# SkyTNT/midi-model

Hardware: AMD Instinct MI355X
Metric: MIDI events/sec, training step (fwd+bwd+clip+AdamW), tv2o-medium, seq=2048 (higher is better)
Workload: dtype bf16; 1 GPU; tv2o-medium bf16 training step, per-GPU batch 16 x 2048 events x 8 tokens (BASELINE.json configs[1]); random-init weights, synthetic events; global_batch=16, seq_len=2048, parallelism=dp1, accumulate_grad_batches=1, optimizer=AdamW bf16-true + global-norm clip 1.0

## Files before the change

### include/midihip.h

```cpp
#ifndef MIDIHIP_H
#define MIDIHIP_H
#include <stdint.h>
#ifdef __cplusplus
extern "C" {
#endif

#define MH_F32 0
#define MH_BF16 1

#define MH_OK 0
#define MH_ERR_ARG (-1)
#define MH_ERR_LAUNCH (-2)
#define MH_ERR_UNSUPPORTED (-3)

const char* mh_last_error(void);
int mh_version(void);
int mh_ab_builds(void);
int mh_set_option(const char* name, int value);
int mh_get_option(const char* name);

int mh_gemm_nt(const void* A, int64_t lda, const void* B, int64_t ldb, void* C, int64_t ldc, const void* R,
               int64_t ldr, int64_t M, int64_t N, int64_t K, float alpha, float beta, int dtype, int splitk,
               void* workspace, void* stream);
int mh_gemm(const void* A, int64_t lda, int transA, const void* B, int64_t ldb, int transB, void* C, int64_t ldc,
// ... 28 lines not shown
int mh_scale_cols_batched(const int64_t* jobs, int njobs, int K, int dtype, void* stream);
int mh_gemm_splitk_reduce(const void* workspace, void* C, int64_t ldc, const void* R, int64_t ldr, int64_t M,
                          int64_t N, int splitk, float alpha, float beta, int dtype, void* stream);
#define MH_SKINNY_PLAIN 0
#define MH_SKINNY_GATEUP 1
int mh_gemm_skinny(const void* A, int64_t lda, const void* W, int64_t ldw, void* C, int64_t ldc, const void* R,
                   int64_t ldr, int mode, float norm_eps, const int64_t* row_ids, const int64_t* res_ids, int64_t M,
                   int64_t N, int64_t K, int dtype, void* stream);
int mh_transpose(const void* in, int64_t ldi, void* out, int64_t ldo, int64_t rows, int64_t cols, int dtype,
                 void* stream);

int mh_embed_sum_fwd(const int64_t* tok, const void* table, void* out, int64_t M, int T, int64_t V, int D,
                     int dtype, void* stream);
int mh_concat_tok_fwd(const void* hidden, const int64_t* tok, int64_t ldtok, const void* table, void* out,
                      int64_t M, int T, int64_t V, int D, int dtype, void* stream);
int mh_embed_scatter_bwd(const int64_t* tok, int64_t ldtok, int T, const void* dout, int rows_per_m, int jstride,
                         int j0, float* dtable_f32, int64_t M, int64_t V, int D, int64_t pad_id, int dtype,
                         void* stream);
int mh_embed_segment_bwd(const int64_t* src_rows, const int64_t* seg_start, const void* dout, int64_t ld,
                         float* dtable_f32, int64_t V, int D, int64_t n_occ, int64_t pad_id, int dtype, void* stream);
int mh_embed_segment_sum(const int64_t* src_rows, const int64_t* seg_start, const void* rows, int64_t ld, float* sum_f32,
                         int64_t ldsum, int64_t V, int D, int64_t n_occ, int dtype, void* stream);
int mh_embed_split_hi_lo(const float* s, void* hi, void* lo, int64_t n, int dtype, void* stream);
int mh_embed_table_norm_bwd(const void* t_hi, const void* t_lo, const void* e, const float* rstd, float* acc32, int64_t V, int D,
                            int64_t pad_id, int dtype, void* stream);
int mh_token_segments_chunk(void);
int mh_token_segments(const int64_t* tok, int64_t ldtok, int64_t n_rows, int n_cols, int64_t V, int64_t row_mul,
                      int64_t col_mul, int64_t add, int64_t* src_rows, int64_t* seg_start, int32_t* work, void* stream);
int mh_cast_from_f32(const float* src, void* dst, int64_t n, int accumulate, int dtype, void* stream);
int mh_copy_rows(const void* src, int64_t src_ld, void* dst, int64_t dst_ld, int64_t M, int D, int accumulate,
                 int dtype, void* stream);

int mh_collate_windows(const int16_t* tokens, int64_t n_events, const int64_t* win_start, const int64_t* win_len,
                       int64_t* out, int64_t B, int64_t L, int T, int64_t pad_id, void* stream);

int mh_augment_piece_stats(const int16_t* tokens, const int64_t* piece_off, int64_t n_pieces, const int32_t* tab,
                           int32_t* stats, void* stream);
int mh_augment_collate_windows(const int16_t* tokens, int64_t n_events, const int64_t* win_start, const int64_t* win_len,
                               const int64_t* win_piece, const int32_t* shifts, const int32_t* stats, const int32_t* tab,
                               int64_t* out, int64_t B, int64_t L, int T, int64_t pad_id, void* stream);

int mh_rmsnorm_fwd(const void* x, const void* w, void* y, float* rstd, int64_t M, int D, float eps, int dtype,
                   void* stream);
int mh_rmsnorm_bwd_blocks(int64_t M);
int mh_rmsnorm_bwd(const void* x, const void* w, const float* rstd, const void* dy, const void* dres, void* dx,
                   float* dw_partial, int64_t M, int D, int dtype, void* stream);
int mh_colsum(float* partial , int64_t nblk, void* out, int D, int accumulate, int dtype, void* stream);

int mh_rope(void* qkv, const float* cos_t, const float* sin_t, int64_t M, int64_t S, int64_t pos0, int H, int hd,
            int dir, int dtype, void* stream);

// ... 7 lines not shown
                const float* cos_t, const float* sin_t, int dtype, void* stream);
int mh_attn_bwd_o(const void* qkv, const void* o, const void* dout, const float* lse, float* delta, void* dqkv, int64_t B,
                  int64_t S, int H, float scale, const float* cos_t, const float* sin_t, int dtype, void* stream);
int mh_attn_bwd_o_scaled(const void* qkv, const void* o, const void* dout, const float* lse, float* delta, void* dqkv,
                         const float* rowscale, int64_t B, int64_t S, int H, float scale, const float* cos_t, const float* sin_t,
                         int dtype, void* stream);
int mh_attn_fwd_timeline(const void* qkv, void* o, float* lse, int64_t B, int64_t S, int H, float scale, int lazy,
                         uint32_t* stamps, void* stream);
int mh_attn_fwd_plain(const void* qkv, void* o, float* lse, int64_t B, int64_t S, int H, float scale, int dtype,
                      void* stream);
int mh_attn_bwd_plain(const void* qkv, const void* dout, const float* lse, const float* delta, void* dqkv, int64_t B,
                      int64_t S, int H, float scale, int dtype, void* stream);

int mh_tokattn_fwd(const void* qkv, void* o, int64_t N, int T, int H, float scale, const float* cos_t, const float* sin_t,
                   int dtype, void* stream);
int mh_tokattn_bwd(const void* qkv, const void* dout, void* dqkv, int64_t N, int T, int H, float scale, const float* cos_t,
                   const float* sin_t, int dtype, void* stream);
int mh_tokattn_bwd_scaled(const void* qkv, const void* dout, void* dqkv, const float* rowscale, int64_t N, int T, int H, float scale,
                          const float* cos_t, const float* sin_t, int dtype, void* stream);
int mh_tokattn_fwd_rows(const void* zc, const int64_t* ids, int64_t ldid, int64_t tab0, int64_t V, void* o, int64_t N, int H,
                        float scale, const float* cos_t, const float* sin_t, int dtype, void* stream);
int mh_tokattn_bwd_rows(const void* zc, const int64_t* ids, int64_t ldid, int64_t tab0, int64_t V, const void* dout, void* dz,
                        void* dz_hid, const float* rowscale, int64_t N, int H, float scale, const float* cos_t, const float* sin_t,
                        int dtype, void* stream);

int mh_swiglu_fwd(const void* gu, void* a, int64_t M, int I, int dtype, void* stream);
int mh_swiglu_bwd(const void* gu, const void* da, void* dgu, int64_t M, int I, int dtype, void* stream);

int mh_cross_entropy(const void* logits, int64_t ldl, const int64_t* target, float* row_loss, void* dlogits,
                     const float* scale_dev, int64_t* argmax_out, int64_t R, int V, int64_t ignore, int dtype,
                     void* stream);
int mh_sum_f32(const float* x, int64_t n, float* out, void* stream);
int mh_count_valid(const int64_t* target, int64_t n, int64_t ignore, float* count, float* inv, void* stream);

int mh_sumsq(const void* g, int64_t n, float* partial1024, float* out, int accumulate, int dtype, void* stream);
int mh_clip_coef(const float* sumsq, float max_norm, float* coef, float* norm, void* stream);
int mh_adamw(void* p, const void* g, void* m, void* v, int64_t n, float lr, float beta1, float beta2, float eps,
             float weight_decay, float bias_corr1, float bias_corr2, const float* coef_dev, int dtype, void* stream);
int mh_adamw_master(float* p32, void* p_lo, const float* g32, float* m, float* v, int64_t n, float lr, float beta1,
                    float beta2, float eps, float weight_decay, float bias_corr1, float bias_corr2, const float* coef_dev,
                    int dtype_lo, void* stream);
int mh_grad_fold_f32(const void* src, float* dst, int64_t n, int accumulate, int dtype, void* stream);

int mh_kv_append(void* qkv, const float* cos_t, const float* sin_t, void* kcache, void* vcache, int64_t B, int H,
                 int hd, int64_t Lmax, int64_t pos, const int32_t* pos_dev, int dtype, void* stream);
int mh_attn_decode(const void* qkv, const void* kcache, const void* vcache, void* o, int64_t B, int H, int hd,
                   int64_t Lmax, int64_t len, float scale, const int32_t* pos_dev, int dtype, void* stream);
// ... 43 lines not shown
```

### midi-model_amd/csrc/attention_small.hip

```cpp
#include "common.h"

#define DISPATCH_T(dtype, CALL)                                    \
  do {                                                             \
    if ((dtype) == MH_BF16) { using T = bf16; CALL; }              \
    else if ((dtype) == MH_F32) { using T = float; CALL; }         \
    else { mh_set_error("bad dtype %d", (int)(dtype)); return MH_ERR_ARG; } \
  } while (0)

template <typename T> __device__ inline void ld4(const T* p, float (&o)[4]);
template <> __device__ inline void ld4<float>(const float* p, float (&o)[4]) {
  f32x4 v = *reinterpret_cast<const f32x4*>(p);
  o[0] = v[0]; o[1] = v[1]; o[2] = v[2]; o[3] = v[3];
}
template <> __device__ inline void ld4<bf16>(const bf16* p, float (&o)[4]) {
  bf16x4 v = *reinterpret_cast<const bf16x4*>(p);
  o[0] = (float)v[0]; o[1] = (float)v[1]; o[2] = (float)v[2]; o[3] = (float)v[3];
}
template <typename T> __device__ inline void st4(T* p, const float (&o)[4]);
template <> __device__ inline void st4<float>(float* p, const float (&o)[4]) {
  *reinterpret_cast<f32x4*>(p) = f32x4{o[0], o[1], o[2], o[3]};
}
template <> __device__ inline void st4<bf16>(bf16* p, const float (&o)[4]) {
  bf16x4 v;
  v[0] = (bf16)o[0]; v[1] = (bf16)o[1]; v[2] = (bf16)o[2]; v[3] = (bf16)o[3];
// ... 40 lines not shown
template <typename T>
__device__ inline void rope4(float (&x)[4], const float (&c)[2], const float (&s)[2], float dir, bool round) {
#pragma unroll
  for (int e = 0; e < 2; ++e) {
    const float x1 = x[e], x2 = x[e + 2], sn = dir * s[e];
    const float r1 = x1 * c[e] - x2 * sn, r2 = x2 * c[e] + x1 * sn;
    x[e] = round ? rnd<T>(r1) : r1;
    x[e + 2] = round ? rnd<T>(r2) : r2;
  }
}

template <typename T>
__device__ inline void rope_row(float (&x)[4], const float* rope_c, const float* rope_s, int t, int lane, float dir,
                                bool round) {
  const float rc[2] = {rope_c[t * 128 + 2 * lane], rope_c[t * 128 + 2 * lane + 1]};
  const float rs[2] = {rope_s[t * 128 + 2 * lane], rope_s[t * 128 + 2 * lane + 1]};
  rope4<T>(x, rc, rs, dir, round);
}

struct TokRows {
  const int64_t* ids;
  int64_t ldid, tab0;
  int V;
};
template <int TN>
__device__ inline int tok_row_lane(const TokRows& tr, int64_t n, int lane) {
  int id = 0;
  if (lane >= 1 && lane < TN) id = (int)tr.ids[n * tr.ldid + lane - 1];
  return id < 0 ? 0 : (id >= tr.V ? tr.V - 1 : id);
}

template <typename T, int TN, bool IND = false>
__global__ __launch_bounds__(256) void tokattn_fwd_kernel(const T* __restrict__ qkv, T* __restrict__ o, int64_t NH, int Tn,
                                                          int H, float scale, const float* __restrict__ cos_t,
                                                          const float* __restrict__ sin_t, TokRows tr = TokRows{}) {
  static_assert(!IND || TN == TK, "row indirection: the octet form only");
  const int lane = threadIdx.x & 63;
  const int64_t D = (int64_t)H * 256, D3 = 3 * D;
  __shared__ float rope_c[TK * 128], rope_s[TK * 128];
  const bool rot = cos_t != nullptr;
  if (rot) {
    for (int i = threadIdx.x; i < Tn * 128; i += 256) {
      rope_c[i] = rnd<T>(cos_t[i]);
      rope_s[i] = rnd<T>(sin_t[i]);
    }
    __syncthreads();
// ... 82 lines not shown
  static_assert(!IND || TN == TK, "row indirection: the octet form only");
  const int lane = threadIdx.x & 63;
  const int64_t D = (int64_t)H * 256, D3 = 3 * D;
  __shared__ float rope_c[TK * 128], rope_s[TK * 128];
  const bool rot = cos_t != nullptr;
  if (rot) {
    for (int i = threadIdx.x; i < Tn * 128; i += 256) {
      rope_c[i] = rnd<T>(cos_t[i]);
      rope_s[i] = rnd<T>(sin_t[i]);
    }
    __syncthreads();
  }
  for (int64_t w = (int64_t)blockIdx.x * 4 + (threadIdx.x >> 6); w < NH; w += (int64_t)gridDim.x * 4) {
    const int64_t n = w / H;
    const int h = (int)(w - n * H);
    const int64_t off = (int64_t)h * 256;
    const T* base = qkv + (IND ? 0 : n * Tn * D3) + off;
    T* ob = dqkv + n * Tn * D3 + off;
    T* ob0 = (IND && dq_hid != nullptr) ? dq_hid + n * D3 + off : ob;
    float k[TK][4], v[TK][4], dk[TK][4], dv[TK][4];
    RawRow<T> qraw[TN ? TN : 1], doraw[TN ? TN : 1];
    int idl = 0;
    if constexpr (IND) idl = tok_row_lane<TN>(tr, n, lane);
    const int64_t rs_row = IND ? (lane == 0 ? n : tr.tab0 + idl) : n * Tn + lane;
    const float rs_lane = (rowscale != nullptr && lane < Tn) ? rowscale[rs_row] : 1.f;
#pragma unroll
    for (int t = 0; t < TK; ++t)
#pragma unroll
      for (int e = 0; e < 4; ++e) dk[t][e] = dv[t][e] = 0.f;
    if constexpr (TN != 0) {
      RawRow<T> kraw[TN ? TN : 1], vraw[TN ? TN : 1];
      int64_t roff[TN ? TN : 1];
      if constexpr (IND) {
        roff[0] = n * D3;
#pragma unroll
        for (int t = 1; t < TN; ++t) roff[t] = (tr.tab0 + __builtin_amdgcn_readlane(idl, t)) * D3;
      } else {
#pragma unroll
        for (int t = 0; t < TN; ++t) roff[t] = t * D3;
      }
#pragma unroll
      for (int t = 0; t < TN; ++t) {
        kraw[t] = ldraw<T>(base + roff[t] + D, lane);
        vraw[t] = ldraw<T>(base + roff[t] + 2 * D, lane);
      }
#pragma unroll
// ... 69 lines not shown
      const float inv = 1.f / den;
      float dsum = 0.f;
#pragma unroll
      for (int j = 0; j <= i; ++j) {
        p[j] *= inv;
        dsum += p[j] * dp[j];
      }
#pragma unroll
      for (int j = 0; j <= i; ++j) {
        const float ds = p[j] * (dp[j] - dsum) * scale;
#pragma unroll
        for (int e = 0; e < 4; ++e) {
          dq[e] += ds * k[j][e];
          dk[j][e] += ds * q[e];
          dv[j][e] += p[j] * dO[e];
        }
      }
      if (rot) rope_row<T>(dq, rope_c, rope_s, i, lane, -1.f, false);
      if (rowscale != nullptr) {
        const float rsc = __shfl(rs_lane, i, 64);
#pragma unroll
        for (int e = 0; e < 4; ++e) dq[e] *= rsc;
      }
      stp<T>((i == 0 ? ob0 : ob + i * D3), lane, dq);
    }
#pragma unroll
    for (int t = 0; t < TK; ++t) {
      if (TN ? t < TN : t < Tn) {
        if (rot) rope_row<T>(dk[t], rope_c, rope_s, t, lane, -1.f, false);
        if (rowscale != nullptr) {
          const float rsc = __shfl(rs_lane, t, 64);
#pragma unroll
          for (int e = 0; e < 4; ++e) {
            dk[t][e] *= rsc;
            dv[t][e] *= rsc;
          }
        }
        T* orow = t == 0 ? ob0 : ob + t * D3;
        stp<T>(orow + D, lane, dk[t]);
        stp<T>(orow + 2 * D, lane, dv[t]);
      }
    }
  }
}

extern "C" int mh_tokattn_fwd(const void* qkv, void* o, int64_t N, int Tn, int H, float scale, const float* cos_t,
                              const float* sin_t, int dtype, void* stream) {
  MH_REQUIRE(N > 0 && Tn >= 1 && Tn <= TK && H >= 1, "tokattn_fwd: bad shape N=%ld T=%d H=%d", (long)N, Tn, H);
  const int64_t NH = N * H;
  int64_t g = (NH + 3) / 4;
  if (g > 32768) g = 32768;
  if (Tn == TK)
    DISPATCH_T(dtype, (tokattn_fwd_kernel<T, TK><<<(int)g, 256, 0, (hipStream_t)stream>>>((const T*)qkv, (T*)o, NH, Tn, H, scale,
                                                                                          cos_t, sin_t)));
  else
    DISPATCH_T(dtype, (tokattn_fwd_kernel<T, 0><<<(int)g, 256, 0, (hipStream_t)stream>>>((const T*)qkv, (T*)o, NH, Tn, H, scale,
                                                                                         cos_t, sin_t)));
  MH_LAUNCH_CHECK();
  return MH_OK;
}

thread_local int g_tokattn_bwd_batched = 1;
static int tokattn_bwd_any(const void* qkv, const void* dout, void* dqkv, const float* rowscale, int64_t N, int Tn, int H, float scale,
// ... 23 lines not shown
  MH_REQUIRE(rowscale != nullptr, "tokattn_bwd_scaled: rowscale is NULL");
  return tokattn_bwd_any(qkv, dout, dqkv, rowscale, N, Tn, H, scale, cos_t, sin_t, dtype, stream);
}

static int tokattn_rows_check(const void* zc, const int64_t* ids, int64_t ldid, int64_t tab0, int64_t V, int64_t N, int H) {
  MH_REQUIRE(zc != nullptr && ids != nullptr && ldid >= TK - 1 && tab0 >= N && V > 0 && V < (1ll << 31) && N > 0 && H >= 1,
             "tokattn_rows: bad arguments N=%ld H=%d V=%ld tab0=%ld ldid=%ld", (long)N, H, (long)V, (long)tab0, (long)ldid);
  return MH_OK;
}
extern "C" int mh_tokattn_fwd_rows(const void* zc, const int64_t* ids, int64_t ldid, int64_t tab0, int64_t V, void* o, int64_t N,
                                   int H, float scale, const float* cos_t, const float* sin_t, int dtype, void* stream) {
  if (int rc = tokattn_rows_check(zc, ids, ldid, tab0, V, N, H)) return rc;
  const int64_t NH = N * H;
  int64_t g = (NH + 3) / 4;
  if (g > 32768) g = 32768;
  const TokRows tr{ids, ldid, tab0, (int)V};
  DISPATCH_T(dtype, (tokattn_fwd_kernel<T, TK, true><<<(int)g, 256, 0, (hipStream_t)stream>>>((const T*)zc, (T*)o, NH, TK, H, scale,
                                                                                             cos_t, sin_t, tr)));
  MH_LAUNCH_CHECK();
  return MH_OK;
}
extern "C" int mh_tokattn_bwd_rows(const void* zc, const int64_t* ids, int64_t ldid, int64_t tab0, int64_t V, const void* dout,
                                   void* dz, void* dz_hid, const float* rowscale, int64_t N, int H, float scale,
                                   const float* cos_t, const float* sin_t, int dtype, void* stream) {
  if (int rc = tokattn_rows_check(zc, ids, ldid, tab0, V, N, H)) return rc;
  MH_REQUIRE(dout != nullptr && dz != nullptr, "tokattn_bwd_rows: null gradient buffer");
  const int64_t NH = N * H;
  int64_t g = (NH + 3) / 4;
  if (g > 32768) g = 32768;
  const TokRows tr{ids, ldid, tab0, (int)V};
  if (g_tokattn_bwd_batched)
    DISPATCH_T(dtype, (tokattn_bwd_kernel<T, TK, true, true><<<(int)g, 256, 0, (hipStream_t)stream>>>(
                          (const T*)zc, (const T*)dout, (T*)dz, NH, TK, H, scale, cos_t, sin_t, rowscale, tr, (T*)dz_hid)));
  else
    DISPATCH_T(dtype, (tokattn_bwd_kernel<T, TK, false, true><<<(int)g, 256, 0, (hipStream_t)stream>>>(
                          (const T*)zc, (const T*)dout, (T*)dz, NH, TK, H, scale, cos_t, sin_t, rowscale, tr, (T*)dz_hid)));
  MH_LAUNCH_CHECK();
  return MH_OK;
}

template <typename T>
__global__ __launch_bounds__(256) void kv_append_kernel(T* __restrict__ qkv, const float* __restrict__ cos_t,
                                                        const float* __restrict__ sin_t, T* __restrict__ kc,
                                                        T* __restrict__ vc, int64_t B, int H, int hd, int64_t Lmax,
                                                        int64_t pos, const int32_t* __restrict__ pos_dev) {
  if (pos_dev != nullptr) pos = *pos_dev;
  if (pos >= Lmax) return;
  const int half = hd / 2;
  const int64_t total = B * H * half;
  const int64_t D = (int64_t)H * hd;
  for (int64_t it = (int64_t)blockIdx.x * 256 + threadIdx.x; it < total; it += (int64_t)gridDim.x * 256) {
    const int i = (int)(it % half);
    const int64_t bh = it / half;
// ... 763 lines not shown
```

### midi-model_amd/csrc/elementwise.hip

```cpp
#include "common.h"

#define DISPATCH_T(dtype, CALL)                                    \
  do {                                                             \
    if ((dtype) == MH_BF16) { using T = bf16; CALL; }              \
    else if ((dtype) == MH_F32) { using T = float; CALL; }         \
    else { mh_set_error("bad dtype %d", (int)(dtype)); return MH_ERR_ARG; } \
  } while (0)

static inline int grid_for(int64_t items, int per_block, int cap = 1 << 20) {
  int64_t g = (items + per_block - 1) / per_block;
  if (g < 1) g = 1;
  if (g > cap) g = cap;
  return (int)g;
}

template <typename T>
__global__ __launch_bounds__(256) void embed_sum_fwd_kernel(const int64_t* __restrict__ tok, const T* __restrict__ table,
                                                            T* __restrict__ out, int64_t M, int TT, int D, int64_t V) {
  constexpr int N = Pack<T>::N;
  const int lane = threadIdx.x & 63;
  const int64_t wave0 = (int64_t)blockIdx.x * 4 + (threadIdx.x >> 6);
  for (int64_t m = wave0; m < M; m += (int64_t)gridDim.x * 4) {
    constexpr int TMAXI = 8;
    int64_t ids[TMAXI];
// ... 158 lines not shown
      if (c < D) {
        if (own) {
#pragma unroll
          for (int e = 0; e < N; e += 4) {
            float4 t = *reinterpret_cast<float4*>(dst + c + e);
            t.x += acc[ch][e]; t.y += acc[ch][e + 1]; t.z += acc[ch][e + 2]; t.w += acc[ch][e + 3];
            *reinterpret_cast<float4*>(dst + c + e) = t;
          }
        } else {
#pragma unroll
          for (int e = 0; e < N; ++e) atomicAdd(dst + c + e, acc[ch][e]);
        }
#pragma unroll
        for (int e = 0; e < N; ++e) acc[ch][e] = 0.f;
      }
    }
  };
#pragma unroll 1
  for (int64_t p0 = p_beg; p0 < p_end; p0 += RW) {
  const int cnt = (p_end - p0 < RW) ? (int)(p_end - p0) : RW;
  int row_lo = 0, row_hi = 0, my_id = -1;
  if (lane < cnt) {
    const int64_t p = p0 + lane;
    const int64_t r = src[p];
    row_lo = (int)(uint32_t)r;
    row_hi = (int)(r >> 32);
    my_id = owner(p);
  }
#pragma unroll
  for (int j0 = 0; j0 < RW; j0 += G) {
    if (j0 < cnt) {
      Pack<T> buf[G][NCH];
      int idj[G];
#pragma unroll
      for (int g = 0; g < G; ++g) {
        idj[g] = __builtin_amdgcn_readlane(my_id, j0 + g);
        const int64_t row = ((int64_t)__builtin_amdgcn_readlane(row_hi, j0 + g) << 32) |
                            (uint32_t)__builtin_amdgcn_readlane(row_lo, j0 + g);
        if (idj[g] >= 0 && idj[g] != pad_id) {
#pragma unroll
          for (int ch = 0; ch < NCH; ++ch) {
            const int c = (ch * 64 + lane) * N;
            if (c < D) buf[g][ch] = ld16(dout + row * ld + c);
          }
        }
      }
#pragma unroll
// ... 93 lines not shown
  for (int64_t i = (int64_t)blockIdx.x * 256 + threadIdx.x; i < n4; i += (int64_t)gridDim.x * 256) {
    const f32x4 v = *reinterpret_cast<const f32x4*>(s + 4 * i);
    float h[4], l[4];
#pragma unroll
    for (int e = 0; e < 4; ++e) {
      h[e] = rnd<T>(v[e]);
      l[e] = v[e] - h[e];
    }
#pragma unroll
    for (int e = 0; e < 4; ++e) {
      hi[4 * i + e] = from_f<T>(h[e]);
      lo[4 * i + e] = from_f<T>(l[e]);
    }
  }
}
extern "C" int mh_embed_split_hi_lo(const float* s, void* hi, void* lo, int64_t n, int dtype, void* stream) {
  MH_REQUIRE(n > 0 && n % 4 == 0 && s != nullptr && hi != nullptr && lo != nullptr && ((uintptr_t)s & 15) == 0, "embed_split_hi_lo: bad args");
  DISPATCH_T(dtype, (split_hi_lo_kernel<T><<<grid_for(n / 4, 256, 4096), 256, 0, (hipStream_t)stream>>>(s, (T*)hi, (T*)lo, n / 4)));
  MH_LAUNCH_CHECK();
  return MH_OK;
}

template <typename T>
__global__ __launch_bounds__(256) void embed_table_norm_bwd_kernel(const T* __restrict__ t_hi, const T* __restrict__ t_lo,
                                                                   const T* __restrict__ e, const float* __restrict__ rstd,
                                                                   float* __restrict__ acc32, int64_t V, int D, int64_t pad_id) {
  constexpr int N = Pack<T>::N;
  const int lane = threadIdx.x & 63, wv = threadIdx.x >> 6;
  for (int64_t v = (int64_t)blockIdx.x * 4 + wv; v < V; v += (int64_t)gridDim.x * 4) {
    if (v == pad_id) continue;
    const float r = rstd[v];
    float dot = 0.f;
    for (int c = lane * N; c < D; c += 64 * N) {
      const Pack<T> hv = ld16(t_hi + v * D + c), lv = ld16(t_lo + v * D + c), ev = ld16(e + v * D + c);
#pragma unroll
      for (int k = 0; k < N; ++k) dot += (hv.get(k) + lv.get(k)) * ev.get(k);
    }
    const float cf = r * r * wave_sum(dot) / (float)D;
    for (int c = lane * N; c < D; c += 64 * N) {
      const Pack<T> hv = ld16(t_hi + v * D + c), lv = ld16(t_lo + v * D + c), ev = ld16(e + v * D + c);
      float* dst = acc32 + v * D + c;
#pragma unroll
      for (int k = 0; k < N; ++k) dst[k] += (hv.get(k) + lv.get(k)) - ev.get(k) * cf;
    }
  }
}
// ... 24 lines not shown
    if (i < n) {
      const int64_t r = i / ncol;
      atomicAdd(&seg_lds[seg_bucket(tok[r * ld + (i - r * ncol)], V)], 1);
    }
  }
  __syncthreads();
  int32_t* out = cnt + (int64_t)blockIdx.x * (V + 1);
  for (int v = threadIdx.x; v <= V; v += 256) out[v] = seg_lds[v];
}

__global__ __launch_bounds__(256) void token_colscan_kernel(int32_t* __restrict__ cnt, int nb, int V, int32_t* __restrict__ tot) {
  const int v = blockIdx.x * 256 + threadIdx.x;
  if (v > V) return;
  int run = 0;
  for (int b = 0; b < nb; ++b) {
    int32_t* p = cnt + (int64_t)b * (V + 1) + v;
    const int c = *p;
    *p = run;
    run += c;
  }
  tot[v] = run;
}

__global__ __launch_bounds__(256) void token_place_kernel(const int64_t* __restrict__ tok, int64_t ld, int64_t n, int ncol, int V,
                                                          const int32_t* __restrict__ cnt, const int32_t* __restrict__ tot,
                                                          int64_t row_mul, int64_t col_mul, int64_t add,
                                                          int64_t* __restrict__ src_rows, int64_t* __restrict__ seg_start) {
  extern __shared__ int seg_lds[];
  __shared__ int wsum[4];
  const int per = (V + 1 + 255) / 256, v0 = threadIdx.x * per;
  int mine = 0;
  for (int k = 0; k < per; ++k)
    if (v0 + k <= V) mine += tot[v0 + k];
  const int lane = threadIdx.x & 63, wave = threadIdx.x >> 6;
  int inc = mine;
#pragma unroll
  for (int d = 1; d < 64; d <<= 1) {
    const int o = __shfl_up(inc, d);
    if (lane >= d) inc += o;
  }
  if (lane == 63) wsum[wave] = inc;
  __syncthreads();
  int start = inc - mine;
  for (int w = 0; w < wave; ++w) start += wsum[w];
  const int32_t* mycnt = cnt + (int64_t)blockIdx.x * (V + 1);
  for (int k = 0; k < per; ++k) {
    const int v = v0 + k;
    if (v <= V) {
      if (blockIdx.x == 0) seg_start[v] = start;
      seg_lds[v] = start + mycnt[v];
      start += tot[v];
    }
  }
  __syncthreads();
  const int64_t i0 = (int64_t)blockIdx.x * SEG_CH;
#pragma unroll
  for (int s = 0; s < SEG_CH / 256; ++s) {
    const int64_t i = i0 + s * 256 + threadIdx.x;
    if (i < n) {
      const int64_t r = i / ncol;
      const int64_t j = i - r * ncol;
      const int p = atomicAdd(&seg_lds[seg_bucket(tok[r * ld + j], V)], 1);
      src_rows[p] = r * row_mul + j * col_mul + add;
    }
  }
}

extern "C" int mh_token_segments_chunk(void) { return SEG_CH; }

extern "C" int mh_token_segments(const int64_t* tok, int64_t ldtok, int64_t n_rows, int n_cols, int64_t V, int64_t row_mul,
                                 int64_t col_mul, int64_t add, int64_t* src_rows, int64_t* seg_start, int32_t* work,
                                 void* stream) {
  MH_REQUIRE(tok && src_rows && seg_start && work, "token_segments: null argument");
  MH_REQUIRE(n_rows > 0 && n_cols > 0 && ldtok >= n_cols && V > 0 && V < 16000, "token_segments: bad shape rows=%ld cols=%d V=%ld",
             (long)n_rows, n_cols, (long)V);
  const int64_t n = n_rows * n_cols;
  MH_REQUIRE(n < (1ll << 31), "token_segments: %ld occurrences (positions are 32-bit)", (long)n);
  const int nb = (int)((n + SEG_CH - 1) / SEG_CH);
  int32_t* tot = work + (int64_t)nb * (V + 1);
  const size_t lds = (size_t)(V + 1) * sizeof(int);
  hipStream_t st = (hipStream_t)stream;
  token_hist_kernel<<<nb, 256, lds, st>>>(tok, ldtok, n, n_cols, (int)V, work);
  token_colscan_kernel<<<(int)((V + 1 + 255) / 256), 256, 0, st>>>(work, nb, (int)V, tot);
  token_place_kernel<<<nb, 256, lds, st>>>(tok, ldtok, n, n_cols, (int)V, work, tot, row_mul, col_mul, add, src_rows, seg_start);
  MH_LAUNCH_CHECK();
  return MH_OK;
}

template <typename T>
__global__ __launch_bounds__(256) void cast_from_f32_kernel(const float* __restrict__ src, T* __restrict__ dst, int64_t n,
                                                            int accumulate) {
  for (int64_t i = (int64_t)blockIdx.x * 256 + threadIdx.x; i < n; i += (int64_t)gridDim.x * 256) {
    float v = src[i];
    if (accumulate) v += to_f(dst[i]);
    dst[i] = from_f<T>(v);
  }
}

extern "C" int mh_cast_from_f32(const float* src, void* dst, int64_t n, int accumulate, int dtype, void* stream) {
  MH_REQUIRE(n > 0, "cast_from_f32: empty");
  DISPATCH_T(dtype, (cast_from_f32_kernel<T><<<grid_for(n, 256, 4096), 256, 0, (hipStream_t)stream>>>(src, (T*)dst, n,
                                                                                                     accumulate)));
  MH_LAUNCH_CHECK();
  return MH_OK;
}

template <typename T>
// ... 589 lines not shown
```

### midi-model_amd/engine.py

```python
from __future__ import annotations

import math
from dataclasses import dataclass, field
from typing import Callable, List, NamedTuple, Optional

import os

import torch

from . import ops, tokfirst


@dataclass
class StackSpec:
    name: str
    D: int
    H: int
    I: int
    L: int
    eps: float
    theta: float
    kind: str

    @property
# ... 317 lines not shown
    del dz2
    dx2 = _empty((M, D), dx)
    ops.rmsnorm_bwd_folded(keep.x2, keep.rstd2, t2, dx, dx2)
    do = t2
    ops.gemm_nt(dx2, lw.wo, do, tb=True)
    linear_wgrad(dx2, keep.o, lg.wo, accumulate)
    return dx2, do


class TokFirstGrads(NamedTuple):
    dhidden: torch.Tensor
    dtable32: torch.Tensor


def tok_first_backward(spec: StackSpec, lw: LayerTensors, lg: LayerTensors, fold, keep: LayerSaved, first: tokfirst.TokFirst,
                       dx: torch.Tensor, nseq: int, rope: RopeTable, accumulate: bool) -> TokFirstGrads:
    M, D = dx.shape
    H, T = spec.H, tokfirst.TN
    N, V = first.hidden.shape[0], first.table.shape[0]
    assert N == nseq and M == N * T
    wq_n, wgu_n = fold
    xc, rstd_c, zc = keep.x, keep.rstd1, keep.qkv
    dres, do = _folded_mlp_o_backward(spec, lw, lg, wgu_n, keep, dx, accumulate)
    dz = _empty((M, 3 * D), dx)
    dzc = _empty((N + 2 * V, 3 * D), dx)
    tokfirst.tokattn_bwd_rows(zc, first.ids, N, V, do, dz, dzc[:N], rstd_c, N, H, spec.scale, rope.cos, rope.sin)
    del do
    src, seg, vseg, vstart = tokfirst.occurrence_lists(first.ids[:, : T - 1], V, T, 1)
    S = _empty((V, 3 * D), dx, torch.float32)
    tokfirst.segment_sum_fixed_order(src, vseg, vstart, dz, S)
    del dz
    tokfirst.split_hi_lo(S, dzc[N:N + V], dzc[N + V:])
    del S
    tc = _empty((N + 2 * V, D), dx)
    ops.gemm_nt(dzc, wq_n, tc, tb=True)
    ops.wgrad_folded(dzc, xc, lg.wqkv, lw.n1, lw.wqkv, lg.n1, accumulate)
    del dzc
    dres_h = _empty((N, D), dx)
    ops.copy_rows(dres, T * D, dres_h, D, N, D)
    dhid = _empty((N, D), dx)
    ops.rmsnorm_bwd_folded(xc[:N], rstd_c[:N], tc[:N], dres_h, dhid)
    acc32 = torch.zeros((V, D), dtype=torch.float32, device=dx.device)
    ops.embed_segment_bwd(src, seg, dres, D, acc32, first.pad_id)
    tokfirst.table_norm_bwd(tc[N:N + V], tc[N + V:], xc[N:N + V], rstd_c[N:N + V], acc32, first.pad_id)
    return TokFirstGrads(dhid, acc32)


def stack_forward(spec: StackSpec, W: StackTensors, x: torch.Tensor, nseq: int, slen: int, rope: RopeTable,
                  save: bool, kv_out: Optional[list] = None, lean: bool = False, folded=None,
                  first: Optional[tokfirst.TokFirst] = None):
    _check_heads(spec)
    M, D = x.shape
    assert M == nseq * slen
    rope.ensure(slen)
    if runs_folded(spec, x, save, kv_out, folded is not None):
        if folded is None:
# ... 216 lines not shown
```

### midi-model_amd/tokfirst.py

```python
from __future__ import annotations

import os
from typing import NamedTuple, Optional

import torch

from .lib import lib
from .ops import _p, _rowmajor, _stream, dt

TN = 8


class TokFirst(NamedTuple):
    hidden: torch.Tensor
    ids: torch.Tensor
    table: torch.Tensor
    pad_id: int


def table_first_ok(spec, first: Optional[TokFirst], slen: int) -> bool:
    return (first is not None and spec.kind == "token" and slen == TN and first.hidden.is_cuda
            and first.hidden.dtype == torch.bfloat16 and first.table.shape[0] >= 4 and os.environ.get("MH_TOK_TABLE", "1") != "0")


def tokattn_fwd_rows(zc, ids, tab0: int, V: int, o, N: int, H: int, scale: float, cos_t, sin_t):
    assert ids.dtype == torch.int64 and ids.stride(1) == 1 and ids.shape[1] >= TN - 1 and zc.shape[0] >= tab0 + V
    lib().call("mh_tokattn_fwd_rows", _p(zc), _p(ids), ids.stride(0), tab0, V, _p(o), N, H, scale, _p(cos_t), _p(sin_t), dt(zc),
               _stream())
    return o


def tokattn_bwd_rows(zc, ids, tab0: int, V: int, dout, dz, dz_hid, rowscale, N: int, H: int, scale: float, cos_t, sin_t):
    assert ids.dtype == torch.int64 and ids.stride(1) == 1 and ids.shape[1] >= TN - 1 and zc.shape[0] >= tab0 + V
    assert dz.is_contiguous() and (dz_hid is None or dz_hid.is_contiguous())
    assert rowscale is None or (rowscale.dtype == torch.float32 and rowscale.is_contiguous() and rowscale.numel() >= tab0 + V)
    lib().call("mh_tokattn_bwd_rows", _p(zc), _p(ids), ids.stride(0), tab0, V, _p(dout), _p(dz), _p(dz_hid), _p(rowscale), N, H, scale,
               _p(cos_t), _p(sin_t), dt(zc), _stream())
    return dz


def segment_sum(src_rows, seg_start, rows, out_f32):
    V, D = out_f32.shape
    assert src_rows.dtype == torch.int64 and seg_start.dtype == torch.int64 and seg_start.numel() == V + 1 and src_rows.is_contiguous()
    assert out_f32.dtype == torch.float32 and rows.shape[1] == D
    lib().call("mh_embed_segment_sum", _p(src_rows), _p(seg_start), _p(rows), _rowmajor(rows), _p(out_f32), _rowmajor(out_f32), V, D,
               src_rows.numel(), dt(rows), _stream())
    return out_f32


SEG_OWN = 1024


def occurrence_lists(ids: torch.Tensor, V: int, row_mul: int, add: int):
    N, C = ids.shape
    dev = ids.device
    R = N * row_mul
    rows = torch.arange(N, device=dev)[:, None] * row_mul + torch.arange(C, device=dev)[None, :] + add
    key, _ = torch.sort((ids * R + rows).reshape(-1))
    src = key % R
    seg = torch.searchsorted(key, torch.arange(V + 1, device=dev) * R)
    n = N * C
    Vb = V + (n + SEG_OWN - 1) // SEG_OWN
    pieces = torch.clamp((seg[1:] - seg[:-1] + SEG_OWN - 1) // SEG_OWN, min=1)
    vstart = torch.zeros(V + 1, dtype=torch.int64, device=dev)
    vstart[1:] = torch.cumsum(pieces, 0)
    j = torch.arange(Vb + 1, device=dev)
    v = torch.clamp(torch.searchsorted(vstart, j, right=True) - 1, max=V - 1)
    vseg = torch.minimum(seg[v] + (j - vstart[v]) * SEG_OWN, seg[v + 1])
    return src.contiguous(), seg.contiguous(), vseg.contiguous(), vstart


def segment_sum_fixed_order(src, vseg, vstart, rows, out_f32):
    V, D = out_f32.shape
    Vb = vseg.numel() - 1
    part = torch.zeros((Vb, D), dtype=torch.float32, device=rows.device)
    segment_sum(src, vseg, rows, part)
    out_f32.zero_()
    return segment_sum(torch.arange(Vb, device=rows.device), vstart, part, out_f32)


def split_hi_lo(s_f32, hi, lo):
    assert s_f32.dtype == torch.float32 and s_f32.is_contiguous() and hi.is_contiguous() and lo.is_contiguous()
    assert hi.shape == s_f32.shape == lo.shape and hi.dtype == lo.dtype
    lib().call("mh_embed_split_hi_lo", _p(s_f32), _p(hi), _p(lo), s_f32.numel(), dt(hi), _stream())


def table_norm_bwd(t_hi, t_lo, table, rstd, acc32, pad_id: int):
    V, D = table.shape
    assert t_hi.shape == t_lo.shape == (V, D) and acc32.shape == (V, D) and acc32.dtype == torch.float32 and rstd.shape == (V,)
    assert t_hi.is_contiguous() and t_lo.is_contiguous() and table.is_contiguous() and acc32.is_contiguous() and rstd.is_contiguous()
    lib().call("mh_embed_table_norm_bwd", _p(t_hi), _p(t_lo), _p(table), _p(rstd), _p(acc32), V, D, pad_id, dt(table), _stream())
    return acc32
```

Before: 368,800 events/s.

## Scatter token-attention grads into sorted slots and fuse piece-sum with hi/lo split

After: 370,000 events/s, median of 6. No clear change (+0.3%).

```diff
diff --git a/include/midihip.h b/include/midihip.h
--- a/include/midihip.h
+++ b/include/midihip.h
@@ -74,11 +74,16 @@
 int mh_embed_segment_sum(const int64_t* src_rows, const int64_t* seg_start, const void* rows, int64_t ld, float* sum_f32,
                          int64_t ldsum, int64_t V, int D, int64_t n_occ, int dtype, void* stream);
 int mh_embed_split_hi_lo(const float* s, void* hi, void* lo, int64_t n, int dtype, void* stream);
+int mh_embed_piece_sum(const int64_t* piece_first, const float* part, int64_t ldp, float* s_f32, void* hi, void* lo, int64_t V, int D,
+                       int dtype, void* stream);
 int mh_embed_table_norm_bwd(const void* t_hi, const void* t_lo, const void* e, const float* rstd, float* acc32, int64_t V, int D,
                             int64_t pad_id, int dtype, void* stream);
 int mh_token_segments_chunk(void);
 int mh_token_segments(const int64_t* tok, int64_t ldtok, int64_t n_rows, int n_cols, int64_t V, int64_t row_mul,
                       int64_t col_mul, int64_t add, int64_t* src_rows, int64_t* seg_start, int32_t* work, void* stream);
+int mh_token_occurrence_lists(const int64_t* tok, int64_t ldtok, int64_t n_rows, int n_cols, int64_t V, int64_t row_mul, int64_t add,
+                              int64_t* src_rows, int64_t* seg_start, int64_t* piece_start, int64_t* piece_first, int64_t* slot,
+                              int32_t* work, void* stream);
 int mh_cast_from_f32(const float* src, void* dst, int64_t n, int accumulate, int dtype, void* stream);
 int mh_copy_rows(const void* src, int64_t src_ld, void* dst, int64_t dst_ld, int64_t M, int D, int accumulate,
                  int dtype, void* stream);
@@ -132,7 +137,7 @@
                         float scale, const float* cos_t, const float* sin_t, int dtype, void* stream);
 int mh_tokattn_bwd_rows(const void* zc, const int64_t* ids, int64_t ldid, int64_t tab0, int64_t V, const void* dout, void* dz,
                         void* dz_hid, const float* rowscale, int64_t N, int H, float scale, const float* cos_t, const float* sin_t,
-                        int dtype, void* stream);
+                        const int64_t* dst_slot, int64_t ldslot, int dtype, void* stream);
 
 int mh_swiglu_fwd(const void* gu, void* a, int64_t M, int I, int dtype, void* stream);
 int mh_swiglu_bwd(const void* gu, const void* da, void* dgu, int64_t M, int I, int dtype, void* stream);
diff --git a/midi-model_amd/csrc/attention_small.hip b/midi-model_amd/csrc/attention_small.hip
--- a/midi-model_amd/csrc/attention_small.hip
+++ b/midi-model_amd/csrc/attention_small.hip
@@ -86,6 +86,8 @@
   const int64_t* ids;
   int64_t ldid, tab0;
   int V;
+  const int64_t* slot = nullptr;
+  int64_t ldslot = 0, n_slot = 0;
 };
 template <int TN>
 __device__ inline int tok_row_lane(const TokRows& tr, int64_t n, int lane) {
@@ -214,6 +216,20 @@
     RawRow<T> qraw[TN ? TN : 1], doraw[TN ? TN : 1];
     int idl = 0;
     if constexpr (IND) idl = tok_row_lane<TN>(tr, n, lane);
+    int sli = 0;
+    if constexpr (IND) {
+      if (tr.slot != nullptr) {
+        int64_t sl = 0;
+        if (lane >= 1 && lane < TN) sl = tr.slot[n * tr.ldslot + lane - 1];
+        sli = (int)(sl < 0 ? 0 : (sl >= tr.n_slot ? tr.n_slot - 1 : sl));
+      }
+    }
+    auto out_row = [&](int t) -> T* {
+      if constexpr (IND) {
+        if (tr.slot != nullptr) return dqkv + off + (int64_t)__builtin_amdgcn_readlane(sli, t) * D3;
+      }
+      return ob + t * D3;
+    };
     const int64_t rs_row = IND ? (lane == 0 ? n : tr.tab0 + idl) : n * Tn + lane;
     const float rs_lane = (rowscale != nullptr && lane < Tn) ? rowscale[rs_row] : 1.f;
 #pragma unroll
@@ -329,7 +345,7 @@
 #pragma unroll
         for (int e = 0; e < 4; ++e) dq[e] *= rsc;
       }
-      stp<T>((i == 0 ? ob0 : ob + i * D3), lane, dq);
+      stp<T>((i == 0 ? ob0 : out_row(i)), lane, dq);
     }
 #pragma unroll
     for (int t = 0; t < TK; ++t) {
@@ -343,9 +359,9 @@
             dv[t][e] *= rsc;
           }
         }
-        T* orow = t == 0 ? ob0 : ob + t * D3;
-        stp<T>(orow + D, lane, dk[t]);
-        stp<T>(orow + 2 * D, lane, dv[t]);
+        T* out = t == 0 ? ob0 : out_row(t);
+        stp<T>(out + D, lane, dk[t]);
+        stp<T>(out + 2 * D, lane, dv[t]);
       }
     }
   }
@@ -415,13 +431,15 @@
 }
 extern "C" int mh_tokattn_bwd_rows(const void* zc, const int64_t* ids, int64_t ldid, int64_t tab0, int64_t V, const void* dout,
                                    void* dz, void* dz_hid, const float* rowscale, int64_t N, int H, float scale,
-                                   const float* cos_t, const float* sin_t, int dtype, void* stream) {
+                                   const float* cos_t, const float* sin_t, const int64_t* dst_slot, int64_t ldslot, int dtype,
+                                   void* stream) {
   if (int rc = tokattn_rows_check(zc, ids, ldid, tab0, V, N, H)) return rc;
   MH_REQUIRE(dout != nullptr && dz != nullptr, "tokattn_bwd_rows: null gradient buffer");
+  MH_REQUIRE(dst_slot == nullptr || (dz_hid != nullptr && ldslot >= TK - 1), "tokattn_bwd_rows: dst_slot needs dz_hid and ldslot >= 7");
   const int64_t NH = N * H;
   int64_t g = (NH + 3) / 4;
   if (g > 32768) g = 32768;
-  const TokRows tr{ids, ldid, tab0, (int)V};
+  const TokRows tr{ids, ldid, tab0, (int)V, dst_slot, ldslot, N * (TK - 1)};
   if (g_tokattn_bwd_batched)
     DISPATCH_T(dtype, (tokattn_bwd_kernel<T, TK, true, true><<<(int)g, 256, 0, (hipStream_t)stream>>>(
                           (const T*)zc, (const T*)dout, (T*)dz, NH, TK, H, scale, cos_t, sin_t, rowscale, tr, (T*)dz_hid)));
diff --git a/midi-model_amd/csrc/elementwise.hip b/midi-model_amd/csrc/elementwise.hip
--- a/midi-model_amd/csrc/elementwise.hip
+++ b/midi-model_amd/csrc/elementwise.hip
@@ -204,7 +204,7 @@
   int row_lo = 0, row_hi = 0, my_id = -1;
   if (lane < cnt) {
     const int64_t p = p0 + lane;
-    const int64_t r = src[p];
+    const int64_t r = src != nullptr ? src[p] : p;
     row_lo = (int)(uint32_t)r;
     row_hi = (int)(r >> 32);
     my_id = owner(p);
@@ -344,6 +344,46 @@
 }
 
 template <typename T>
+__global__ __launch_bounds__(256) void piece_sum_split_kernel(const int64_t* __restrict__ piece_first, const float* __restrict__ part,
+                                                              int64_t ldp, int D, float* __restrict__ s_f32, T* __restrict__ hi,
+                                                              T* __restrict__ lo) {
+  const int64_t v = blockIdx.x;
+  const int c = (blockIdx.y * 256 + threadIdx.x) * 4;
+  if (c >= D) return;
+  const int64_t k0 = piece_first[v], k1 = piece_first[v + 1];
+  float acc[4] = {0.f, 0.f, 0.f, 0.f};
+  for (int64_t k = k0; k < k1; ++k) {
+    const f32x4 t = *reinterpret_cast<const f32x4*>(part + k * ldp + c);
+#pragma unroll
+    for (int e = 0; e < 4; ++e) acc[e] += t[e];
+  }
+  float s[4];
+#pragma unroll
+  for (int e = 0; e < 4; ++e) s[e] = 0.f + acc[e];
+  if (s_f32 != nullptr) *reinterpret_cast<f32x4*>(s_f32 + v * D + c) = f32x4{s[0], s[1], s[2], s[3]};
+  if (hi != nullptr) {
+#pragma unroll
+    for (int e = 0; e < 4; ++e) {
+      const float h = rnd<T>(s[e]);
+      hi[v * D + c + e] = from_f<T>(h);
+      lo[v * D + c + e] = from_f<T>(s[e] - h);
+    }
+  }
+}
+extern "C" int mh_embed_piece_sum(const int64_t* piece_first, const float* part, int64_t ldp, float* s_f32, void* hi, void* lo, int64_t V,
+                                  int D, int dtype, void* stream) {
+  MH_REQUIRE(V > 0 && V < (1ll << 31) && D > 0 && D % 4 == 0 && ldp % 4 == 0 && ldp >= D && piece_first != nullptr && part != nullptr &&
+                 (hi == nullptr) == (lo == nullptr) && (s_f32 != nullptr || hi != nullptr) &&
+                 (((uintptr_t)part | (uintptr_t)s_f32) & 15) == 0,
+             "embed_piece_sum: bad args V=%ld D=%d ldp=%ld", (long)V, D, (long)ldp);
+  MH_REQUIRE((D + 1023) / 1024 < 65536, "embed_piece_sum: too many columns");
+  DISPATCH_T(dtype, (piece_sum_split_kernel<T><<<dim3((unsigned)V, (unsigned)((D + 1023) / 1024)), 256, 0, (hipStream_t)stream>>>(
+                        piece_first, part, ldp, D, s_f32, (T*)hi, (T*)lo)));
+  MH_LAUNCH_CHECK();
+  return MH_OK;
+}
+
+template <typename T>
 __global__ __launch_bounds__(256) void embed_table_norm_bwd_kernel(const T* __restrict__ t_hi, const T* __restrict__ t_lo,
                                                                    const T* __restrict__ e, const float* __restrict__ rstd,
                                                                    float* __restrict__ acc32, int64_t V, int D, int64_t pad_id) {
@@ -414,12 +454,8 @@
   tot[v] = run;
 }
 
-__global__ __launch_bounds__(256) void token_place_kernel(const int64_t* __restrict__ tok, int64_t ld, int64_t n, int ncol, int V,
-                                                          const int32_t* __restrict__ cnt, const int32_t* __restrict__ tot,
-                                                          int64_t row_mul, int64_t col_mul, int64_t add,
-                                                          int64_t* __restrict__ src_rows, int64_t* __restrict__ seg_start) {
-  extern __shared__ int seg_lds[];
-  __shared__ int wsum[4];
+__device__ inline void seg_chunk_cursors(const int32_t* __restrict__ cnt, const int32_t* __restrict__ tot, int V, int* seg_lds, int* wsum,
+                                         int64_t* __restrict__ seg_start) {
   const int per = (V + 1 + 255) / 256, v0 = threadIdx.x * per;
   int mine = 0;
   for (int k = 0; k < per; ++k)
@@ -445,6 +481,15 @@
     }
   }
   __syncthreads();
+}
+
+__global__ __launch_bounds__(256) void token_place_kernel(const int64_t* __restrict__ tok, int64_t ld, int64_t n, int ncol, int V,
+                                                          const int32_t* __restrict__ cnt, const int32_t* __restrict__ tot,
+                                                          int64_t row_mul, int64_t col_mul, int64_t add,
+                                                          int64_t* __restrict__ src_rows, int64_t* __restrict__ seg_start) {
+  extern __shared__ int seg_lds[];
+  __shared__ int wsum[4];
+  seg_chunk_cursors(cnt, tot, V, seg_lds, wsum, seg_start);
   const int64_t i0 = (int64_t)blockIdx.x * SEG_CH;
 #pragma unroll
   for (int s = 0; s < SEG_CH / 256; ++s) {
@@ -454,6 +499,96 @@
       const int64_t j = i - r * ncol;
       const int p = atomicAdd(&seg_lds[seg_bucket(tok[r * ld + j], V)], 1);
       src_rows[p] = r * row_mul + j * col_mul + add;
+    }
+  }
+}
+
+__global__ __launch_bounds__(256) void token_place_stable_kernel(const int64_t* __restrict__ tok, int64_t ld, int64_t n, int ncol, int V,
+                                                                 const int32_t* __restrict__ cnt, const int32_t* __restrict__ tot,
+                                                                 int64_t row_mul, int64_t add, int64_t* __restrict__ src_rows,
+                                                                 int64_t* __restrict__ seg_start, int64_t* __restrict__ slot) {
+  extern __shared__ int seg_lds[];
+  __shared__ int wsum[4];
+  seg_chunk_cursors(cnt, tot, V, seg_lds, wsum, seg_start);
+  const int lane = threadIdx.x & 63, wave = threadIdx.x >> 6;
+  const int64_t i0 = (int64_t)blockIdx.x * SEG_CH;
+#pragma unroll 1
+  for (int s = 0; s < SEG_CH / 256; ++s) {
+    const int64_t i = i0 + s * 256 + threadIdx.x;
+    int64_t row = 0;
+    int b = -1;
+    if (i < n) {
+      const int64_t r = i / ncol;
+      const int64_t j = i - r * ncol;
+      b = seg_bucket(tok[r * ld + j], V);
+      row = r * row_mul + j + add;
+    }
+    int rank = 0, same = 0, leader = lane;
+    unsigned long long todo = __ballot(b >= 0);
+    while (todo != 0) {
+      const int first = __ffsll(todo) - 1;
+      const int fb = __shfl(b, first, 64);
+      const unsigned long long m = __ballot(b == fb);
+      if (b == fb) {
+        rank = __popcll(m & ((1ull << lane) - 1ull));
+        same = __popcll(m);
+        leader = first;
+      }
+      todo &= ~m;
+    }
+    int base = 0;
+    for (int w = 0; w < 4; ++w) {
+      if (wave == w && b >= 0 && lane == leader) {
+        base = seg_lds[b];
+        seg_lds[b] = base + same;
+      }
+      __syncthreads();
+    }
+    base = __shfl(base, leader, 64);
+    if (b >= 0) {
+      const int p = base + rank;
+      src_rows[p] = row;
+      slot[i] = p;
+    }
+  }
+}
+
+__global__ __launch_bounds__(256) void token_pieces_kernel(const int64_t* __restrict__ seg_start, int V, int n_piece,
+                                                           int64_t* __restrict__ piece_start, int64_t* __restrict__ piece_first) {
+  __shared__ int wsum[4];
+  auto pieces_of = [&](int v) {
+    const int64_t c = seg_start[v + 1] - seg_start[v];
+    return c <= SEG_OWN ? 1 : (int)((c + SEG_OWN - 1) / SEG_OWN);
+  };
+  const int per = (V + 255) / 256, v0 = threadIdx.x * per;
+  int mine = 0;
+  for (int k = 0; k < per; ++k)
+    if (v0 + k < V) mine += pieces_of(v0 + k);
+  const int lane = threadIdx.x & 63, wave = threadIdx.x >> 6;
+  int inc = mine;
+#pragma unroll
+  for (int d = 1; d < 64; d <<= 1) {
+    const int o = __shfl_up(inc, d);
+    if (lane >= d) inc += o;
+  }
+  if (lane == 63) wsum[wave] = inc;
+  __syncthreads();
+  int start = inc - mine;
+  for (int w = 0; w < wave; ++w) start += wsum[w];
+  for (int k = 0; k < per; ++k) {
+    const int v = v0 + k;
+    if (v >= V) break;
+    const int pc = pieces_of(v);
+    const int64_t s0 = seg_start[v], s1 = seg_start[v + 1];
+    piece_first[v] = start;
+    for (int q = 0; q < pc && start + q <= n_piece; ++q) {
+      const int64_t at = s0 + (int64_t)q * SEG_OWN;
+      piece_start[start + q] = at < s1 ? at : s1;
+    }
+    start += pc;
+    if (v == V - 1) {
+      piece_first[V] = start;
+      for (int j = start; j <= n_piece; ++j) piece_start[j] = s1;
     }
   }
 }
@@ -475,6 +610,27 @@
   token_hist_kernel<<<nb, 256, lds, st>>>(tok, ldtok, n, n_cols, (int)V, work);
   token_colscan_kernel<<<(int)((V + 1 + 255) / 256), 256, 0, st>>>(work, nb, (int)V, tot);
   token_place_kernel<<<nb, 256, lds, st>>>(tok, ldtok, n, n_cols, (int)V, work, tot, row_mul, col_mul, add, src_rows, seg_start);
+  MH_LAUNCH_CHECK();
+  return MH_OK;
+}
+
+extern "C" int mh_token_occurrence_lists(const int64_t* tok, int64_t ldtok, int64_t n_rows, int n_cols, int64_t V, int64_t row_mul,
+                                        int64_t add, int64_t* src_rows, int64_t* seg_start, int64_t* piece_start,
+                                        int64_t* piece_first, int64_t* slot, int32_t* work, void* stream) {
+  MH_REQUIRE(tok && src_rows && seg_start && piece_start && piece_first && slot && work, "token_occurrence_lists: null argument");
+  MH_REQUIRE(n_rows > 0 && n_cols > 0 && ldtok >= n_cols && row_mul >= n_cols && V > 0 && V < 16000,
+             "token_occurrence_lists: bad shape rows=%ld cols=%d V=%ld row_mul=%ld", (long)n_rows, n_cols, (long)V, (long)row_mul);
+  const int64_t n = n_rows * n_cols;
+  MH_REQUIRE(n < (1ll << 31), "token_occurrence_lists: %ld occurrences (positions are 32-bit)", (long)n);
+  const int nb = (int)((n + SEG_CH - 1) / SEG_CH);
+  const int n_piece = (int)(V + (n + SEG_OWN - 1) / SEG_OWN);
+  int32_t* tot = work + (int64_t)nb * (V + 1);
+  const size_t lds = (size_t)(V + 1) * sizeof(int);
+  hipStream_t st = (hipStream_t)stream;
+  token_hist_kernel<<<nb, 256, lds, st>>>(tok, ldtok, n, n_cols, (int)V, work);
+  token_colscan_kernel<<<(int)((V + 1 + 255) / 256), 256, 0, st>>>(work, nb, (int)V, tot);
+  token_place_stable_kernel<<<nb, 256, lds, st>>>(tok, ldtok, n, n_cols, (int)V, work, tot, row_mul, add, src_rows, seg_start, slot);
+  token_pieces_kernel<<<1, 256, 0, st>>>(seg_start, (int)V, n_piece, piece_start, piece_first);
   MH_LAUNCH_CHECK();
   return MH_OK;
 }
diff --git a/midi-model_amd/engine.py b/midi-model_amd/engine.py
--- a/midi-model_amd/engine.py
+++ b/midi-model_amd/engine.py
@@ -363,16 +363,24 @@
     wq_n, wgu_n = fold
     xc, rstd_c, zc = keep.x, keep.rstd1, keep.qkv
     dres, do = _folded_mlp_o_backward(spec, lw, lg, wgu_n, keep, dx, accumulate)
-    dz = _empty((M, 3 * D), dx)
     dzc = _empty((N + 2 * V, 3 * D), dx)
-    tokfirst.tokattn_bwd_rows(zc, first.ids, N, V, do, dz, dzc[:N], rstd_c, N, H, spec.scale, rope.cos, rope.sin)
-    del do
-    src, seg, vseg, vstart = tokfirst.occurrence_lists(first.ids[:, : T - 1], V, T, 1)
-    S = _empty((V, 3 * D), dx, torch.float32)
-    tokfirst.segment_sum_fixed_order(src, vseg, vstart, dz, S)
-    del dz
-    tokfirst.split_hi_lo(S, dzc[N:N + V], dzc[N + V:])
-    del S
+    if tokfirst.sorted_ok(dx):
+        src, seg, vseg, vstart, slot = tokfirst.token_occurrence_lists(first.ids[:, : T - 1], V, T, 1)
+        dz = _empty((N * (T - 1), 3 * D), dx)
+        tokfirst.tokattn_bwd_rows(zc, first.ids, N, V, do, dz, dzc[:N], rstd_c, N, H, spec.scale, rope.cos, rope.sin, dst_slot=slot)
+        del do
+        tokfirst.sorted_rows_sum(vseg, vstart, dz, dzc[N:N + V], dzc[N + V:])
+        del dz
+    else:
+        dz = _empty((M, 3 * D), dx)
+        tokfirst.tokattn_bwd_rows(zc, first.ids, N, V, do, dz, dzc[:N], rstd_c, N, H, spec.scale, rope.cos, rope.sin)
+        del do
+        src, seg, vseg, vstart = tokfirst.occurrence_lists(first.ids[:, : T - 1], V, T, 1)
+        S = _empty((V, 3 * D), dx, torch.float32)
+        tokfirst.segment_sum_fixed_order(src, vseg, vstart, dz, S)
+        del dz
+        tokfirst.split_hi_lo(S, dzc[N:N + V], dzc[N + V:])
+        del S
     tc = _empty((N + 2 * V, D), dx)
     ops.gemm_nt(dzc, wq_n, tc, tb=True)
     ops.wgrad_folded(dzc, xc, lg.wqkv, lw.n1, lw.wqkv, lg.n1, accumulate)
diff --git a/midi-model_amd/tokfirst.py b/midi-model_amd/tokfirst.py
--- a/midi-model_amd/tokfirst.py
+++ b/midi-model_amd/tokfirst.py
@@ -30,21 +30,29 @@
     return o
 
 
-def tokattn_bwd_rows(zc, ids, tab0: int, V: int, dout, dz, dz_hid, rowscale, N: int, H: int, scale: float, cos_t, sin_t):
+def tokattn_bwd_rows(zc, ids, tab0: int, V: int, dout, dz, dz_hid, rowscale, N: int, H: int, scale: float, cos_t, sin_t,
+                     dst_slot=None):
     assert ids.dtype == torch.int64 and ids.stride(1) == 1 and ids.shape[1] >= TN - 1 and zc.shape[0] >= tab0 + V
     assert dz.is_contiguous() and (dz_hid is None or dz_hid.is_contiguous())
     assert rowscale is None or (rowscale.dtype == torch.float32 and rowscale.is_contiguous() and rowscale.numel() >= tab0 + V)
+    if dst_slot is not None:
+        assert dst_slot.dtype == torch.int64 and dst_slot.is_contiguous() and dst_slot.numel() == N * (TN - 1)
+        assert dz_hid is not None and dz.shape[0] >= N * (TN - 1)
+    else:
+        assert dz.shape[0] >= N * TN
     lib().call("mh_tokattn_bwd_rows", _p(zc), _p(ids), ids.stride(0), tab0, V, _p(dout), _p(dz), _p(dz_hid), _p(rowscale), N, H, scale,
-               _p(cos_t), _p(sin_t), dt(zc), _stream())
+               _p(cos_t), _p(sin_t), _p(dst_slot), TN - 1, dt(zc), _stream())
     return dz
 
 
 def segment_sum(src_rows, seg_start, rows, out_f32):
     V, D = out_f32.shape
-    assert src_rows.dtype == torch.int64 and seg_start.dtype == torch.int64 and seg_start.numel() == V + 1 and src_rows.is_contiguous()
+    assert seg_start.dtype == torch.int64 and seg_start.numel() == V + 1
+    assert src_rows is None or (src_rows.dtype == torch.int64 and src_rows.is_contiguous())
     assert out_f32.dtype == torch.float32 and rows.shape[1] == D
+    n_occ = rows.shape[0] if src_rows is None else src_rows.numel()
     lib().call("mh_embed_segment_sum", _p(src_rows), _p(seg_start), _p(rows), _rowmajor(rows), _p(out_f32), _rowmajor(out_f32), V, D,
-               src_rows.numel(), dt(rows), _stream())
+               n_occ, dt(rows), _stream())
     return out_f32
 
 
@@ -70,6 +78,46 @@
     return src.contiguous(), seg.contiguous(), vseg.contiguous(), vstart
 
 
+def sorted_ok(t: torch.Tensor) -> bool:
+    return t.is_cuda and os.environ.get("MH_TOK_SORTED", "1") != "0"
+
+
+def token_occurrence_lists(ids: torch.Tensor, V: int, row_mul: int, add: int):
+    assert ids.dim() == 2 and ids.dtype == torch.int64 and ids.stride(1) == 1 and ids.is_cuda
+    N, C = ids.shape
+    assert row_mul >= C
+    n = N * C
+    Vb = V + (n + SEG_OWN - 1) // SEG_OWN
+    chunk = lib().cdll.mh_token_segments_chunk()
+    dev = ids.device
+    work = torch.empty((((n + chunk - 1) // chunk) + 1) * (V + 1), dtype=torch.int32, device=dev)
+    src = torch.empty(n, dtype=torch.int64, device=dev)
+    slot = torch.empty(n, dtype=torch.int64, device=dev)
+    seg = torch.empty(V + 1, dtype=torch.int64, device=dev)
+    vseg = torch.empty(Vb + 1, dtype=torch.int64, device=dev)
+    vstart = torch.empty(V + 1, dtype=torch.int64, device=dev)
+    lib().call("mh_token_occurrence_lists", _p(ids), ids.stride(0), N, C, V, row_mul, add, _p(src), _p(seg), _p(vseg), _p(vstart),
+               _p(slot), _p(work), _stream())
+    return src, seg, vseg, vstart, slot
+
+
+def piece_sum(vstart, part, s_f32=None, hi=None, lo=None):
+    V = vstart.numel() - 1
+    D = part.shape[1]
+    assert part.dtype == torch.float32 and vstart.dtype == torch.int64 and (hi is None) == (lo is None)
+    assert s_f32 is None or (s_f32.dtype == torch.float32 and s_f32.shape == (V, D) and s_f32.is_contiguous())
+    assert hi is None or (hi.shape == (V, D) == lo.shape and hi.dtype == lo.dtype and hi.is_contiguous() and lo.is_contiguous())
+    lib().call("mh_embed_piece_sum", _p(vstart), _p(part), _rowmajor(part), _p(s_f32), _p(hi), _p(lo), V, D,
+               dt(hi) if hi is not None else dt(part), _stream())
+
+
+def sorted_rows_sum(vseg, vstart, rows_sorted, hi, lo, s_f32=None):
+    Vb = vseg.numel() - 1
+    part = torch.zeros((Vb, rows_sorted.shape[1]), dtype=torch.float32, device=rows_sorted.device)
+    segment_sum(None, vseg, rows_sorted, part)
+    piece_sum(vstart, part, s_f32, hi, lo)
+
+
 def segment_sum_fixed_order(src, vseg, vstart, rows, out_f32):
     V, D = out_f32.shape
     Vb = vseg.numel() - 1
```
